# raynbowy23/RegT-GCN

Hardware: AMD Instinct MI355X
Metric: training steps/sec (graph-snapshots/sec) (higher is better)
Workload: dtype fp32; 1 GPU; cfg3: ONE synthetic regional graph, 100000 nodes / 1000000 edges / 8 regions, F=32, T=12, O=1, hidden=256; RegionalTemporalGCN forward+MSE+backward per snapshot, RMSprop step once per K steps (run.py semantics); gemm_arithmetic=fp32 MFMA (v_mfma_f32_32x32x2_f32), global_nodes=100000, global_edges=1000000, global_regions=8, parallelism=single GPU

## Files before the change

### regt-gcn_amd/csrc/embed.hip

```cpp
#include "kernels.h"

namespace regt {

namespace {

typedef float f32x4 __attribute__((ext_vector_type(4)));

constexpr int EM_ROWS = 128, EM_C = 256, EM_F = 32, EM_K = 2 * EM_F;
constexpr int EM_WS = EM_C + 16;
constexpr int EM_XS = EM_ROWS + 18;
constexpr int EM_W_BYTES = EM_K * EM_WS * 4, EM_X_BYTES = EM_K * EM_XS * 4;
constexpr int EM_LDS = EM_W_BYTES + 2 * EM_X_BYTES;

struct EmbedArgs {
    const float* X; const float* LX;
    const float* A0; const float* Aall;
    const int* node_region;
    const float* bias;
    float* out;
    long M; int T; float ns;
};

__device__ __forceinline__ __amdgpu_buffer_rsrc_t em_rsrc(const void* p, long bytes) {
    return __builtin_amdgcn_make_buffer_rsrc(const_cast<void*>(p), 0, bytes > 0x7ffffff0L ? 0x7ffffff0 : (bytes < 0 ? 0 : (int)bytes), 0x00020000);
}

__global__ __launch_bounds__(512, 2) void embed_fp32_kernel(EmbedArgs a) {
    extern __shared__ __attribute__((aligned(16))) char elds[];
    float* W = reinterpret_cast<float*>(elds);
    float* XB = reinterpret_cast<float*>(elds + EM_W_BYTES);
    const int tid = threadIdx.x, lane = tid & 63, c = lane & 15, g = lane >> 4;
    const int w = __builtin_amdgcn_readfirstlane(tid >> 6), rh = w >> 2, cq = w & 3;
    const long tiles = (a.M + EM_ROWS - 1) / EM_ROWS;
    const unsigned uT = (unsigned)a.T;

    f32x4 px[2], pl[2];
    auto request_rows = [&](long tile) {
        const long m0 = tile * EM_ROWS;
        const long left = a.M - m0;
        const long nv = left < 0 ? 0 : (left < EM_ROWS ? left : EM_ROWS);
        const __amdgpu_buffer_rsrc_t sx = em_rsrc(a.X + m0 * EM_F, nv * EM_F * 4), sl = em_rsrc(a.LX + m0 * EM_F, nv * EM_F * 4);
#pragma unroll
        for (int i = 0; i < 2; ++i) {
            const int off = (tid + 512 * i) * 16;
            px[i] = __builtin_bit_cast(f32x4, __builtin_amdgcn_raw_buffer_load_b128(sx, off, 0, 0));
            pl[i] = __builtin_bit_cast(f32x4, __builtin_amdgcn_raw_buffer_load_b128(sl, off, 0, 0));
        }
    };
    auto park_rows = [&](int buf) {
        float* xb = XB + buf * (EM_K * EM_XS);
#pragma unroll
        for (int i = 0; i < 2; ++i) {
            const int f = tid + 512 * i, row = f >> 3, k0 = 4 * (f & 7);
#pragma unroll
            for (int j = 0; j < 4; ++j) {
                xb[(k0 + j) * EM_XS + row] = px[i][j];
                xb[(EM_F + k0 + j) * EM_XS + row] = pl[i][j];
            }
        }
    };
    float afr[16][4];
    auto stage_weights = [&](int rg) {
        const float* Ar = a.Aall + (long)rg * EM_C * EM_F;
        for (int f = tid; f < EM_C * EM_F / 4; f += 512) {
            const int col = f >> 3, k0 = 4 * (f & 7);
            const float4 v0 = *reinterpret_cast<const float4*>(a.A0 + (long)col * EM_F + k0);
            const float4 v1 = *reinterpret_cast<const float4*>(Ar + (long)col * EM_F + k0);
            W[(k0 + 0) * EM_WS + col] = v0.x; W[(k0 + 1) * EM_WS + col] = v0.y; W[(k0 + 2) * EM_WS + col] = v0.z; W[(k0 + 3) * EM_WS + col] = v0.w;
            W[(EM_F + k0 + 0) * EM_WS + col] = v1.x; W[(EM_F + k0 + 1) * EM_WS + col] = v1.y; W[(EM_F + k0 + 2) * EM_WS + col] = v1.z; W[(EM_F + k0 + 3) * EM_WS + col] = v1.w;
        }
        __syncthreads();
#pragma unroll
        for (int s = 0; s < 16; ++s)
#pragma unroll
            for (int cb = 0; cb < 4; ++cb) afr[s][cb] = W[(4 * s + g) * EM_WS + 64 * cq + 16 * cb + c];
        __syncthreads();
    };
    auto region_of_row = [&](long m) { return a.node_region ? a.node_region[(unsigned)m / uT] : 0; };

    f32x4 bias4[4];
#pragma unroll
    for (int cb = 0; cb < 4; ++cb) bias4[cb] = *reinterpret_cast<const f32x4*>(a.bias + 64 * cq + 16 * cb + 4 * g);

    long tile = blockIdx.x;
    if (tile >= tiles) return;
    int cur_rg = -1, buf = 0;
    auto tile_regions = [&](long t, int* first, int* last) {
        *first = *last = 0;
        if (t < tiles) {
            const long m0 = t * EM_ROWS, m1 = (m0 + EM_ROWS < a.M ? m0 + EM_ROWS : a.M) - 1;
            *first = region_of_row(m0);
            *last = region_of_row(m1);
        }
    };
    int rg_first, rg_last;
    tile_regions(tile, &rg_first, &rg_last);
    request_rows(tile);
    park_rows(0);
#pragma unroll 1
    for (; tile < tiles; tile += gridDim.x) {
        const long m0 = tile * EM_ROWS;
        const long left = a.M - m0;
        const int nv = (int)(left < EM_ROWS ? left : EM_ROWS);
        __syncthreads();
        const long tnext = tile + gridDim.x;
        request_rows(tnext);
        int nrg_first, nrg_last;
        tile_regions(tnext, &nrg_first, &nrg_last);
        const float* xb = XB + buf * (EM_K * EM_XS) + 64 * rh + c;
#pragma unroll 1
        for (int rg = rg_first; rg <= rg_last; ++rg) {
            if (rg != cur_rg) { stage_weights(rg); cur_rg = rg; }
            int lo = 0, hi = nv;
            if (rg_first != rg_last) {
                int l2 = 0, h2 = nv;
                while (l2 < h2) { const int mid = (l2 + h2) >> 1; if (region_of_row(m0 + mid) < rg) l2 = mid + 1; else h2 = mid; }
                lo = l2;
                l2 = lo; h2 = nv;
                while (l2 < h2) { const int mid = (l2 + h2) >> 1; if (region_of_row(m0 + mid) <= rg) l2 = mid + 1; else h2 = mid; }
                hi = l2;
            }
            const __amdgpu_buffer_rsrc_t so = em_rsrc(a.out + (m0 + lo) * EM_C, (long)(hi - lo) * EM_C * 4);
#pragma unroll 1
            for (int rb = 0; rb < 4; ++rb) {
                f32x4 acc[4];
#pragma unroll
                for (int cb = 0; cb < 4; ++cb) acc[cb] = bias4[cb];
#pragma unroll
                for (int s = 0; s < 16; ++s) {
                    const float b = xb[(4 * s + g) * EM_XS + 16 * rb];
#pragma unroll
                    for (int cb = 0; cb < 4; ++cb) acc[cb] = __builtin_amdgcn_mfma_f32_16x16x4f32(afr[s][cb], b, acc[cb], 0, 0, 0);
                }
                const int row = 64 * rh + 16 * rb + c - lo;
                const int voff = row < 0 ? 0x7ffffff0 : row * (EM_C * 4) + (64 * cq + 4 * g) * 4;
#pragma unroll
                for (int cb = 0; cb < 4; ++cb) {
                    f32x4 v = acc[cb];
#pragma unroll
                    for (int i = 0; i < 4; ++i) v[i] = v[i] > 0.f ? v[i] : v[i] * a.ns;
                    __builtin_amdgcn_raw_buffer_store_b128(__builtin_bit_cast(__attribute__((ext_vector_type(4))) unsigned, v), so, voff + 64 * cb, 0, 0);
                }
            }
        }
        park_rows(buf ^ 1);
        buf ^= 1;
        rg_first = nrg_first; rg_last = nrg_last;
    }
}

}

int fused_cus();

bool embed_fp32_ok(long M, int C, int F, int T) { return C == EM_C && F == EM_F && M >= 512L * EM_ROWS && T > 0; }

int launch_embed_fp32(const float* X, const float* LX, const float* A0, const float* Aall, const int* node_region, const float* bias,
                      float* out, long M, int T, int act, float slope, hipStream_t st) {
    REGT_CHECK_ARG(act == ACT_NONE || act == ACT_LRELU || act == ACT_RELU, "embedding kernel: activation %d not covered", act);
    EmbedArgs a{X, LX, A0, Aall, node_region, bias, out, M, T, act == ACT_NONE ? 1.0f : (act == ACT_LRELU ? slope : 0.0f)};
    static bool attr_done = false;
    if (const int rc = set_lds_once(&embed_fp32_kernel, EM_LDS, &attr_done)) return rc;
    const long tiles = (M + EM_ROWS - 1) / EM_ROWS;
    const long cus = fused_cus();
    hipLaunchKernelGGL(embed_fp32_kernel, dim3((unsigned)(tiles < cus ? tiles : cus)), dim3(512), EM_LDS, st, a);
    REGT_CHECK_LAUNCH();
    return REGT_OK;
}

}
```

Before: 62.67 snapshots/s.

## Swizzle embed LDS tile row-major, vectorize B-fragment loads, use fmed3 leaky-ReLU

Changes the staged X/LX tile in LDS from a padded transposed layout to a row-major layout with an XOR swizzle. Each lane can then fetch four K values with one 128-bit LDS read and prefetch the next row block's fragments while the MFMAs run, instead of issuing scalar LDS reads per step. Also folds the bias into the first MFMA and adds a template variant that computes leaky-ReLU with fmed3 when the slope lies in [0,1]. This aims to cut LDS instruction count and latency in the embedding GEMM, but the swizzle must stay conflict-free and correct for both writes and reads.

```diff
diff --git a/regt-gcn_amd/csrc/embed.hip b/regt-gcn_amd/csrc/embed.hip
--- a/regt-gcn_amd/csrc/embed.hip
+++ b/regt-gcn_amd/csrc/embed.hip
@@ -8,8 +8,7 @@
 
 constexpr int EM_ROWS = 128, EM_C = 256, EM_F = 32, EM_K = 2 * EM_F;
 constexpr int EM_WS = EM_C + 16;
-constexpr int EM_XS = EM_ROWS + 18;
-constexpr int EM_W_BYTES = EM_K * EM_WS * 4, EM_X_BYTES = EM_K * EM_XS * 4;
+constexpr int EM_W_BYTES = EM_K * EM_WS * 4, EM_X_BYTES = EM_ROWS * EM_K * 4;
 constexpr int EM_LDS = EM_W_BYTES + 2 * EM_X_BYTES;
 
 struct EmbedArgs {
@@ -25,10 +24,15 @@
     return __builtin_amdgcn_make_buffer_rsrc(const_cast<void*>(p), 0, bytes > 0x7ffffff0L ? 0x7ffffff0 : (bytes < 0 ? 0 : (int)bytes), 0x00020000);
 }
 
+__device__ __forceinline__ int em_swz(int c) { return (((c >> 3) ^ (c >> 2)) & 1) << 3 | (c & 3) << 1 | ((c >> 2) & 1); }
+
+typedef float f32x2 __attribute__((ext_vector_type(2)));
+
+template <bool MAXF>
 __global__ __launch_bounds__(512, 2) void embed_fp32_kernel(EmbedArgs a) {
     extern __shared__ __attribute__((aligned(16))) char elds[];
     float* W = reinterpret_cast<float*>(elds);
-    float* XB = reinterpret_cast<float*>(elds + EM_W_BYTES);
+    char* XB = elds + EM_W_BYTES;
     const int tid = threadIdx.x, lane = tid & 63, c = lane & 15, g = lane >> 4;
     const int w = __builtin_amdgcn_readfirstlane(tid >> 6), rh = w >> 2, cq = w & 3;
     const long tiles = (a.M + EM_ROWS - 1) / EM_ROWS;
@@ -47,15 +51,15 @@
             pl[i] = __builtin_bit_cast(f32x4, __builtin_amdgcn_raw_buffer_load_b128(sl, off, 0, 0));
         }
     };
+    const int park_off = (tid >> 3) * (EM_K * 4) + ((((tid & 7) >> 2) ^ em_swz((tid >> 3) & 15)) << 4) + (tid & 3) * 4;
     auto park_rows = [&](int buf) {
-        float* xb = XB + buf * (EM_K * EM_XS);
+        char* xb = XB + buf * EM_X_BYTES;
 #pragma unroll
         for (int i = 0; i < 2; ++i) {
-            const int f = tid + 512 * i, row = f >> 3, k0 = 4 * (f & 7);
 #pragma unroll
             for (int j = 0; j < 4; ++j) {
-                xb[(k0 + j) * EM_XS + row] = px[i][j];
-                xb[(EM_F + k0 + j) * EM_XS + row] = pl[i][j];
+                *reinterpret_cast<float*>(xb + i * (64 * EM_K * 4) + (park_off ^ (j << 6))) = px[i][j];
+                *reinterpret_cast<float*>(xb + i * (64 * EM_K * 4) + (park_off ^ (j << 6) ^ 32)) = pl[i][j];
             }
         }
     };
@@ -82,6 +86,11 @@
 #pragma unroll
     for (int cb = 0; cb < 4; ++cb) bias4[cb] = *reinterpret_cast<const f32x4*>(a.bias + 64 * cq + 16 * cb + 4 * g);
 
+    const int frag_off = (64 * rh + c) * (EM_K * 4) + (((4 * g) ^ em_swz(c)) << 4);
+
+    float inf = __builtin_inff();
+    asm("" : "+s"(inf));
+
     long tile = blockIdx.x;
     if (tile >= tiles) return;
     int cur_rg = -1, buf = 0;
@@ -107,7 +116,7 @@
         request_rows(tnext);
         int nrg_first, nrg_last;
         tile_regions(tnext, &nrg_first, &nrg_last);
-        const float* xb = XB + buf * (EM_K * EM_XS) + 64 * rh + c;
+        const char* xb = XB + buf * EM_X_BYTES;
 #pragma unroll 1
         for (int rg = rg_first; rg <= rg_last; ++rg) {
             if (rg != cur_rg) { stage_weights(rg); cur_rg = rg; }
@@ -121,24 +130,37 @@
                 hi = l2;
             }
             const __amdgpu_buffer_rsrc_t so = em_rsrc(a.out + (m0 + lo) * EM_C, (long)(hi - lo) * EM_C * 4);
+            f32x4 bq[4];
+#pragma unroll
+            for (int sq = 0; sq < 4; ++sq) bq[sq] = *reinterpret_cast<const f32x4*>(xb + (frag_off ^ (sq << 4)));
 #pragma unroll 1
             for (int rb = 0; rb < 4; ++rb) {
                 f32x4 acc[4];
+                const int nxt = ((rb + 1) & 3) * (16 * EM_K * 4);
 #pragma unroll
-                for (int cb = 0; cb < 4; ++cb) acc[cb] = bias4[cb];
+                for (int sq = 0; sq < 4; ++sq) {
 #pragma unroll
-                for (int s = 0; s < 16; ++s) {
-                    const float b = xb[(4 * s + g) * EM_XS + 16 * rb];
+                    for (int e = 0; e < 4; ++e) {
 #pragma unroll
-                    for (int cb = 0; cb < 4; ++cb) acc[cb] = __builtin_amdgcn_mfma_f32_16x16x4f32(afr[s][cb], b, acc[cb], 0, 0, 0);
+                        for (int cb = 0; cb < 4; ++cb)
+                            acc[cb] = __builtin_amdgcn_mfma_f32_16x16x4f32(afr[4 * sq + e][cb], bq[sq][e], sq + e == 0 ? bias4[cb] : acc[cb], 0, 0, 0);
+                    }
+                    bq[sq] = *reinterpret_cast<const f32x4*>(xb + nxt + (frag_off ^ (sq << 4)));
+                    __builtin_amdgcn_sched_barrier(0);
                 }
                 const int row = 64 * rh + 16 * rb + c - lo;
                 const int voff = row < 0 ? 0x7ffffff0 : row * (EM_C * 4) + (64 * cq + 4 * g) * 4;
 #pragma unroll
                 for (int cb = 0; cb < 4; ++cb) {
                     f32x4 v = acc[cb];
+                    if (MAXF) {
+                        const f32x2 n01 = f32x2{v[0], v[1]} * a.ns, n23 = f32x2{v[2], v[3]} * a.ns;
+                        v = f32x4{__builtin_amdgcn_fmed3f(v[0], n01[0], inf), __builtin_amdgcn_fmed3f(v[1], n01[1], inf),
+                                  __builtin_amdgcn_fmed3f(v[2], n23[0], inf), __builtin_amdgcn_fmed3f(v[3], n23[1], inf)};
+                    } else {
 #pragma unroll
-                    for (int i = 0; i < 4; ++i) v[i] = v[i] > 0.f ? v[i] : v[i] * a.ns;
+                        for (int i = 0; i < 4; ++i) v[i] = v[i] > 0.f ? v[i] : v[i] * a.ns;
+                    }
                     __builtin_amdgcn_raw_buffer_store_b128(__builtin_bit_cast(__attribute__((ext_vector_type(4))) unsigned, v), so, voff + 64 * cb, 0, 0);
                 }
             }
@@ -159,11 +181,14 @@
                       float* out, long M, int T, int act, float slope, hipStream_t st) {
     REGT_CHECK_ARG(act == ACT_NONE || act == ACT_LRELU || act == ACT_RELU, "embedding kernel: activation %d not covered", act);
     EmbedArgs a{X, LX, A0, Aall, node_region, bias, out, M, T, act == ACT_NONE ? 1.0f : (act == ACT_LRELU ? slope : 0.0f)};
-    static bool attr_done = false;
-    if (const int rc = set_lds_once(&embed_fp32_kernel, EM_LDS, &attr_done)) return rc;
+    static bool attr_done[2] = {false, false};
+    const bool maxf = a.ns >= 0.0f && a.ns <= 1.0f;
+    if (const int rc = maxf ? set_lds_once(&embed_fp32_kernel<true>, EM_LDS, &attr_done[1]) : set_lds_once(&embed_fp32_kernel<false>, EM_LDS, &attr_done[0])) return rc;
     const long tiles = (M + EM_ROWS - 1) / EM_ROWS;
     const long cus = fused_cus();
-    hipLaunchKernelGGL(embed_fp32_kernel, dim3((unsigned)(tiles < cus ? tiles : cus)), dim3(512), EM_LDS, st, a);
+    const dim3 grid((unsigned)(tiles < cus ? tiles : cus));
+    if (maxf) hipLaunchKernelGGL(embed_fp32_kernel<true>, grid, dim3(512), EM_LDS, st, a);
+    else hipLaunchKernelGGL(embed_fp32_kernel<false>, grid, dim3(512), EM_LDS, st, a);
     REGT_CHECK_LAUNCH();
     return REGT_OK;
 }
```

After: 61.77 snapshots/s. 1.4% lower.
